# nadeemlab/DeepLIIF

Hardware: AMD Instinct MI355X
Metric: 512x512 tiles/s train-step (5G+5D) (higher is better)
Workload: dtype bf16; 1 GPU; DeepLIIF train step, 5x Resnet-9block G + 5x NLayerD(n=4), GAN+SmoothL1+Adam (BASELINE configs[2] per GPU); tile=512x512x3, batch_per_gpu=8, global_batch=8, norm=instance, precision_policy=bf16, parallelism=dp1, rccl_ranks=1, backend=nccl, streams=3

## Files before the change

deepliif_amd/_lib.py:

```python
import ctypes as C
import os

_HERE = os.path.dirname(os.path.abspath(__file__))
LIB_PATH = os.environ.get('DEEPLIIF_AMD_LIB') or os.path.join(_HERE, 'libdeepliif_hip.so')
LIB_PATH_F16 = os.environ.get('DEEPLIIF_AMD_LIB_F16') or os.path.join(_HERE, 'libdeepliif_hip_f16.so')
HALF_BF16, HALF_FP16 = 0, 1

DL_F32, DL_BF16 = 0, 1
PREC_BF16, PREC_BF16X3 = 1, 3
ACT_NONE, ACT_RELU, ACT_LRELU, ACT_TANH, ACT_SIGMOID = 0, 1, 2, 3, 4
PAD_ZERO, PAD_REFLECT, PAD_REPLICATE = 0, 1, 2
FOLD_SRC_F32 = 0x100
NORM_INSTANCE, NORM_BATCH = 0, 1
LOSS_BCE_LOGITS, LOSS_MSE, LOSS_SMOOTH_L1, LOSS_L1, LOSS_LINEAR = 0, 1, 2, 3, 4
MAX_TAPS, MAX_PHASES = 64, 4
WGRAD_MULTI_MAX = 24
DL_VERSION = 118

i32 = C.c_int32


class ConvDesc(C.Structure):
    _fields_ = [('N', i32), ('Hi', i32), ('Wi', i32), ('Ci', i32), ('in_pstride', i32),
                ('Ho', i32), ('Wo', i32), ('Co', i32), ('out_pstride', i32),
# ... 2 lines not shown
                ('phase_tap_begin', i32 * (MAX_PHASES + 1)), ('phase_kbase', i32 * MAX_PHASES),
                ('tap_dh', C.c_int8 * MAX_TAPS), ('tap_dw', C.c_int8 * MAX_TAPS),
                ('pad_mode', i32), ('w_kstride', i32), ('w_rows', i32), ('act', i32),
                ('in_dtype', i32), ('out_dtype', i32), ('prec', i32), ('splitk', i32), ('in_act', i32), ('bias_n', i32), ('raw_out', i32), ('ci_real', i32), ('in_split', i32)]



class ConvBnStats(C.Structure):
    _fields_ = [('y', C.c_void_p), ('y_pstride', C.c_int32), ('act', C.c_int32),
                ('mean', C.c_void_p), ('rstd', C.c_void_p), ('scale', C.c_void_p), ('shift', C.c_void_p)]

class WgradDesc(C.Structure):
    _fields_ = [('N', i32), ('Hp', i32), ('Wp', i32), ('CAp', i32), ('p_pstride', i32),
                ('Hq', i32), ('Wq', i32), ('CBp', i32), ('q_pstride', i32),
                ('KH', i32), ('KW', i32), ('step', i32), ('pad', i32), ('pad_mode', i32),
                ('CA', i32), ('CB', i32), ('dtype', i32), ('prec', i32), ('splitk', i32), ('accumulate', i32),
                ('q_act', i32), ('p_act', i32), ('pad_w', i32), ('stack_kw', i32), ('p_split', i32), ('q_split', i32)]


class WgradReduceEntry(C.Structure):
    _fields_ = [('slab', C.c_void_p), ('grad', C.c_void_p),
                ('splitk', i32), ('CAp', i32), ('CBp', i32), ('J', i32), ('CA', i32), ('CB', i32), ('KK', i32), ('accumulate', i32), ('stack_kw', i32),
                ('block0', i32), ('nblocks', i32), ('kstride', i32)]


class PackDesc(C.Structure):
    _fields_ = [('A', i32), ('B', i32), ('KH', i32), ('KW', i32), ('row_is_a', i32),
                ('rows_real', i32), ('rows_pad', i32), ('Cc', i32), ('Cc_pad', i32), ('n_phase', i32),
                ('phase_tap_begin', i32 * (MAX_PHASES + 1)), ('phase_kbase', i32 * MAX_PHASES),
                ('tap_kh', C.c_int8 * MAX_TAPS), ('tap_kw', C.c_int8 * MAX_TAPS), ('kstride', i32), ('stack_kw', i32)]


class NormDesc(C.Structure):
    _fields_ = [('N', i32), ('H', i32), ('W', i32), ('Cp', i32), ('C', i32),
                ('y_pstride', i32), ('z_pstride', i32), ('r_pstride', i32),
                ('dtype', i32), ('scope', i32), ('act', i32), ('eps', C.c_float), ('momentum', C.c_float), ('ext_nchunks', i32)]


class RenderThresh(C.Structure):
    _fields_ = [('size_lower', C.c_int64), ('size_upper', C.c_int64), ('marker', C.c_int64), ('od_lower', C.c_int64), ('od_upper', C.c_int64),
                ('has_size_upper', i32), ('has_marker', i32), ('has_od_lower', i32), ('has_od_upper', i32)]


class DropoutDesc(C.Structure):
    _fields_ = [('p', C.c_float), ('seed', C.c_uint64), ('seed_dev', C.c_void_p), ('call_index', C.c_uint32)]

# ... 30 lines not shown
    'dl_conv_wgrad_deferrable': (_i, [C.POINTER(WgradDesc)]),
    'dl_wgrad_slab_floats': (C.c_size_t, [C.POINTER(WgradDesc)]),
    'dl_conv_wgrad_slabs': (_i, [C.POINTER(WgradDesc), _vp, _vp, _vp, _vp, C.POINTER(WgradReduceEntry), _vp]),
    'dl_wgrad_reduce_batch': (_i, [_vp, _i, _i, _vp]),
    'dl_wgrad_plan': (_i, [C.POINTER(WgradDesc), C.POINTER(i32), C.POINTER(i32), C.POINTER(C.c_char_p)]),
    'dl_conv_wgrad_multi': (_i, [C.POINTER(WgradDesc), _i, _vp, _vp, _vp, _vp, C.POINTER(WgradReduceEntry), _vp]),
    'dl_pack_weights': (_i, [C.POINTER(PackDesc), _vp, _vp, _vp, _vp]),
    'dl_pack_job_bytes': (C.c_size_t, []),
    'dl_pack_job_fill': (_i, [C.POINTER(PackDesc), _vp, _vp, _vp, _vp]),
    'dl_pack_batch_blocks': (_i, [_vp, _i, _vp]),
    'dl_pack_weights_batch': (_i, [_vp, _vp, _i, _vp]),
    'dl_spectral_job_bytes': (C.c_size_t, []),
    'dl_spectral_scratch_floats': (C.c_size_t, [_i, _i]),
    'dl_spectral_job_fill': (_i, [_vp, _i, _i, _i, _i, _vp, _vp, _vp, _vp, _vp, _vp, _vp, _vp, _i64, _vp]),
    'dl_spectral_blocks': (_i, [_vp, _i, _i, _vp]),
    'dl_spectral_forward': (_i, [_vp, _i, _vp, _i, _vp, _i, _vp, _i, _vp, _i, _vp]),
    'dl_spectral_backward': (_i, [_vp, _i, _vp, _i, _vp, _i, _vp]),
    'dl_norm_ws_floats': (C.c_size_t, [C.POINTER(NormDesc)]),
    'dl_norm_forward': (_i, [C.POINTER(NormDesc), _vp, _vp, _vp, _vp, _vp, _vp, _vp, _vp, _vp, _vp, _vp, _vp, _vp, _vp]),
    'dl_norm_backward': (_i, [C.POINTER(NormDesc), _vp, _vp, _vp, _vp, _vp, _vp, _vp, _vp, _vp, _vp, _i, _vp, _vp, _vp, _vp]),
    'dl_norm_forward_dropout': (_i, [C.POINTER(NormDesc), _vp, _vp, _vp, _vp, _vp, _vp, _vp, _vp, _vp, _vp, _vp, _vp, _vp, _vp, C.POINTER(DropoutDesc)]),
    'dl_norm_backward_dropout': (_i, [C.POINTER(NormDesc), _vp, _vp, _vp, _vp, _vp, _vp, _vp, _vp, _vp, _vp, _i, _vp, _vp, _vp, _vp,
                                      C.POINTER(DropoutDesc)]),
    'dl_act_forward': (_i, [_i, _i, _vp, _i, _vp, _i, _i64, _i, _vp]),
    'dl_act_backward': (_i, [_i, _i, _vp, _i, _vp, _i, _vp, _i, _i64, _i, _vp]),
    'dl_dropout': (_i, [_i, _vp, _i, _vp, _i, _i64, _i, _f, C.c_uint64, _vp]),
    'dl_dropout_dev': (_i, [_i, _vp, _i, _vp, _i, _i64, _i, C.POINTER(DropoutDesc), _vp]),
    'dl_axpby': (_i, [_i, _f, _vp, _i, _f, _vp, _i, _vp, _i, _i64, _i, _vp]),
    'dl_gate_forward': (_i, [_i, _vp, _i, _vp, _i, _vp, _i, _i64, _i, _vp]),
    'dl_gate_backward': (_i, [_i, _vp, _i, _vp, _i, _vp, _i, _vp, _i, _vp, _i, _i64, _i, _vp]),
    'dl_copy_channels': (_i, [_i, _vp, _i, _i, _vp, _i, _i, _i64, _i, _i, _vp]),
    'dl_channel_sum': (_i, [_i, _vp, _i, _i64, _i, _i, _vp, _i, _vp, _vp]),
    'dl_nchw_to_nhwc': (_i, [_vp, _i, _i, _i, _i, _i, _vp, _i, _i, _i, _vp]),
    'dl_nhwc_to_nchw': (_i, [_i, _vp, _i, _i, _vp, _i, _i, _i, _i, _vp]),
    'dl_conv_narrow_supported': (_i, [_i, _i, _i, _i, _i, _i, _i, _i]),
    'dl_conv_narrow_forward': (_i, [_vp, _i, _i, _i, _i, _i, _vp, _i, _i, _i, _i, _i, _vp, _i, _vp, _i, _i, _vp]),
    'dl_conv_narrow_forward_x3': (_i, [_vp, _i, _i, _i, _i, _i, _vp, _vp, _i, _i, _i, _i, _i, _vp, _i, _vp, _i, _i, _vp]),
    'dl_shift_sum': (_i, [_vp, _i, _i, _i, _i, _i, _i, _i, _i, _vp, _i, _i, _vp, _i, _i, _vp]),
    'dl_shift_stack': (_i, [_i, _vp, _i, _i, _i, _i, _i, _i, _i, _i, _vp, _i, _vp]),
    'dl_reflect_fold': (_i, [_i, _vp, _i, _vp, _i, _i, _i, _i, _i, _i, _vp]),
    'dl_replicate_fold': (_i, [_i, _vp, _i, _vp, _i, _i, _i, _i, _i, _i, _vp]),
    'dl_loss_ws_floats': (C.c_size_t, []),
    'dl_loss': (_i, [_i, _i, _vp, _i, _vp, _i, _f, _i64, _i, _i, _vp, _vp, _i, _f, _vp, _vp]),
    'dl_loss_acc': (_i, [_i, _i, _vp, _i, _vp, _i, _f, _i64, _i, _i, _vp, _f, _i, _vp, _i, _f, _vp, _vp]),
    'dl_upsample2_nearest': (_i, [_i, _i, _vp, _i, _vp, _i, _i, _i, _i, _i, _vp]),
    'dl_kldiv_ws_floats': (C.c_size_t, []),
# ... 60 lines not shown
```

deepliif_amd/csrc/elementwise.hip:

```cpp
#include "common.h"

#define EW_BLOCKS(total) ((int)min((size_t)8192, ((size_t)(total) + 255) / 256))

template <typename T>
__global__ void __launch_bounds__(256) act_fwd_kernel(int act, const T *x, int x_ps, T *y, int y_ps, size_t npix, int Cp) {
    const int cvec = Cp / 8;
    const size_t total = npix * cvec;
    for (size_t i = blockIdx.x * (size_t)blockDim.x + threadIdx.x; i < total; i += (size_t)gridDim.x * blockDim.x) {
        const size_t p = i / cvec;
        const int c0 = (int)(i % cvec) * 8;
        float v[8];
        Vec8<T>::load(x + p * x_ps + c0, v);
#pragma unroll
        for (int k = 0; k < 8; ++k) v[k] = apply_act(act, v[k]);
        Vec8<T>::store(y + p * y_ps + c0, v);
    }
}
template <typename T>
__global__ void __launch_bounds__(256) act_bwd_kernel(int act, const T *dy, int dy_ps, const T *y, int y_ps, T *dx, int dx_ps, size_t npix,
                                                      int Cp) {
    const int cvec = Cp / 8;
    const size_t total = npix * cvec;
    for (size_t i = blockIdx.x * (size_t)blockDim.x + threadIdx.x; i < total; i += (size_t)gridDim.x * blockDim.x) {
        const size_t p = i / cvec;
// ... 210 lines not shown
                Vec8<T>::load(x + p * ps + (cbase + col) * 8, v);
#pragma unroll
                for (int k = 0; k < 8; ++k) s[k] += v[k];
            }
        }
#pragma unroll
        for (int k = 0; k < 8; ++k) red[tid * 9 + k] = s[k];
        __syncthreads();
        if (tid < tpp) {
            float a[8];
#pragma unroll
            for (int k = 0; k < 8; ++k) a[k] = 0.f;
            for (int r = 0; r < rows; ++r)
#pragma unroll
                for (int k = 0; k < 8; ++k) a[k] += red[(r * tpp + tid) * 9 + k];
#pragma unroll
            for (int k = 0; k < 8; ++k) part[(size_t)blockIdx.x * Cp + (cbase + tid) * 8 + k] = a[k];
        }
        __syncthreads();
    }
}
__global__ void __launch_bounds__(256) channel_sum_final_kernel(const float *part, int nblocks, int Cp, int C, float *out, int accumulate) {
    __shared__ float red[8][33];
    const int cl = threadIdx.x & 31, kl = threadIdx.x >> 5;
    const int c = blockIdx.x * 32 + cl;
    float s = 0.f;
    if (c < C)
        for (int b = kl; b < nblocks; b += 8) s += part[(size_t)b * Cp + c];
    red[kl][cl] = s;
    __syncthreads();
    if (kl == 0 && c < C) {
        double a = 0.0;
#pragma unroll
        for (int r = 0; r < 8; ++r) a += (double)red[r][cl];
        out[c] = (accumulate ? out[c] : 0.f) + (float)a;
    }
}
extern "C" int dl_channel_sum(int dtype, const void *x, int ps, int64_t npix, int Cp, int C, float *out, int accumulate, float *ws,
                              void *stream_) {
    hipStream_t stream = (hipStream_t)stream_;
    if (!x || !out || !ws || Cp % 8 || ps % 8) DL_FAIL("dl_channel_sum: bad argument (ws needs %d*Cp floats)", CS_BLOCKS);
    if (dtype == DL_F32) hipLaunchKernelGGL(channel_sum_partial_kernel<float>, dim3(CS_BLOCKS), dim3(256), 0, stream, (const float *)x, ps, (size_t)npix, Cp, ws);
    else hipLaunchKernelGGL(channel_sum_partial_kernel<bf16_t>, dim3(CS_BLOCKS), dim3(256), 0, stream, (const bf16_t *)x, ps, (size_t)npix, Cp, ws);
    DL_CHECK_LAUNCH("dl_channel_sum(partial)");
    hipLaunchKernelGGL(channel_sum_final_kernel, dim3((C + 31) / 32), dim3(256), 0, stream, ws, CS_BLOCKS, Cp, C, out, accumulate);
    DL_CHECK_LAUNCH("dl_channel_sum(final)");
    return 0;
}

#define LOSS_BLOCKS 512
extern "C" size_t dl_loss_ws_floats(void) { return LOSS_BLOCKS; }

template <typename T>
__global__ void __launch_bounds__(256) loss_kernel(int kind, const T *x, int x_ps, const T *target, int t_ps, float tconst, size_t npix, int C,
                                                   float inv_count, T *grad, int g_ps, float gscale, int Cp, float *part) {
    __shared__ float red[4];
    const size_t total = npix * C;
    float acc = 0.f;
    for (size_t i = blockIdx.x * (size_t)blockDim.x + threadIdx.x; i < total; i += (size_t)gridDim.x * blockDim.x) {
        const size_t p = i / C;
        const int c = (int)(i % C);
        const float v = load1<T>(x + p * x_ps + c);
        const float t = target ? load1<T>(target + p * t_ps + c) : tconst;
        float l, g;
        if (kind == DL_LOSS_BCE_LOGITS) {
            const float e = expf(-fabsf(v));
            l = fmaxf(v, 0.f) - v * t + log1pf(e);
            const float sig = v >= 0.f ? 1.f / (1.f + e) : e / (1.f + e);
            g = sig - t;
// ... 554 lines not shown
```

deepliif_amd/csrc/norm.hip:

```cpp
#include "common.h"

struct NormGeom {
    int N, HW, Cp, C;
    int nchunks, ppc;
};

static NormGeom make_geom(const dl_norm_desc *d) {
    NormGeom g;
    g.N = d->N; g.HW = d->H * d->W; g.Cp = d->Cp; g.C = d->C;
    int want = (1024 + d->N - 1) / d->N;
    int maxc = (g.HW + 63) / 64;
    g.nchunks = want < maxc ? want : maxc;
    if (g.nchunks < 1) g.nchunks = 1;
    g.ppc = (g.HW + g.nchunks - 1) / g.nchunks;
    g.nchunks = (g.HW + g.ppc - 1) / g.ppc;
    return g;
}

static NormGeom make_geom_fwd(const dl_norm_desc *d) {
    NormGeom g = make_geom(d);
    if (d->ext_nchunks > 0) { g.nchunks = d->ext_nchunks; g.ppc = 0; }
    return g;
}

// ... 343 lines not shown
        }
        if (bpart) {
#pragma unroll
            for (int k = 0; k < 8; ++k) bred[threadIdx.x * 9 + k] = bs[k];
            __syncthreads();
            if (threadIdx.x < tpp) {
                float a[8];
#pragma unroll
                for (int k = 0; k < 8; ++k) a[k] = 0.f;
                for (int r = 0; r < rows; ++r)
#pragma unroll
                    for (int k = 0; k < 8; ++k) a[k] += bred[(r * tpp + threadIdx.x) * 9 + k];
                float *o = bpart + ((size_t)(n * gridDim.x + blockIdx.x)) * g.Cp + (cbase + threadIdx.x) * 8;
#pragma unroll
                for (int k = 0; k < 8; ++k) o[k] = a[k];
            }
            __syncthreads();
        }
    }
}

__global__ void __launch_bounds__(1024) norm_bias_final_kernel(const float *part, int nparts, int Cp, int C, float *out) {
    __shared__ float red[32][33];
    const int cl = threadIdx.x & 31, kl = threadIdx.x >> 5;
    const int c = blockIdx.x * 32 + cl;
    float s = 0.f;
    if (c < C) {
        float acc[8] = {0.f, 0.f, 0.f, 0.f, 0.f, 0.f, 0.f, 0.f};
        int b = kl;
        for (; b + 7 * 32 < nparts; b += 8 * 32) {
#pragma unroll
            for (int u = 0; u < 8; ++u) acc[u] += part[(size_t)(b + u * 32) * Cp + c];
        }
        for (int u = 0; b < nparts; b += 32, ++u) acc[u & 7] += part[(size_t)b * Cp + c];
        s = ((acc[0] + acc[1]) + (acc[2] + acc[3])) + ((acc[4] + acc[5]) + (acc[6] + acc[7]));
    }
    red[kl][cl] = s;
    __syncthreads();
    if (kl == 0 && c < C) {
        double a = 0.0;
#pragma unroll
        for (int r = 0; r < 32; ++r) a += (double)red[r][cl];
        out[c] += (float)a;
    }
}

static dim3 apply_grid(const NormGeom &g) {
    const int cvec = g.Cp / 8;
    const int rows = 256 / (cvec < 256 ? cvec : 256);
    int bx = (g.HW + rows * 16 - 1) / (rows * 16);
    static const float mul = [] { const char *e = DL_DEV_ENV("DL_NORM_GRID_MUL"); const float v = e ? (float)atof(e) : 1.f; return v > 0.f ? v : 1.f; }();
    const int cap = kBiasPartRows / g.N > 1 ? kBiasPartRows / g.N : 1;
    int want = (int)(cap * mul);
    if (want > cap) want = cap;
    if (bx > want) bx = want;
    if (bx < 1) bx = 1;
    return dim3(bx, g.N);
}

#define DL_NORM_ACT_SWITCH(act_, LAUNCH)                  \
    switch (act_) {                                       \
        case DL_ACT_RELU: LAUNCH(DL_ACT_RELU); break;     \
        case DL_ACT_LRELU: LAUNCH(DL_ACT_LRELU); break;   \
        case DL_ACT_TANH: LAUNCH(DL_ACT_TANH); break;     \
        default: LAUNCH(DL_ACT_NONE); break;              \
    }

// ... 59 lines not shown
    }
    else if (d->dtype == DL_F32) { DL_NORM_ACT_SWITCH(d->act, DL_LAUNCH_APPLY_F32) }
    else { DL_NORM_ACT_SWITCH(d->act, DL_LAUNCH_APPLY_BF16) }
    DL_CHECK_LAUNCH("dl_norm_forward(apply)");
    return 0;
}

extern "C" int dl_norm_forward(const dl_norm_desc *d, const void *y, const float *gamma, const float *beta,
                               float *running_mean, float *running_var, float *mean, float *rstd, float *scale, float *shift,
                               const void *residual, void *z, float *ws, void *z_split, void *stream_) {
    return norm_forward_impl(d, y, gamma, beta, running_mean, running_var, mean, rstd, scale, shift, residual, z, ws, z_split, stream_, nullptr);
}

extern "C" int dl_norm_forward_dropout(const dl_norm_desc *d, const void *y, const float *gamma, const float *beta,
                                       float *running_mean, float *running_var, float *mean, float *rstd, float *scale, float *shift,
                                       const void *residual, void *z, float *ws, void *z_split, void *stream_, const dl_dropout_desc *drop) {
    if (check_drop(drop, "dl_norm_forward_dropout")) return -1;
    return norm_forward_impl(d, y, gamma, beta, running_mean, running_var, mean, rstd, scale, shift, residual, z, ws, z_split, stream_, drop);
}

static int norm_backward_impl(const dl_norm_desc *d, const void *dz, const void *y, const float *gamma,
                              const float *mean, const float *rstd, const float *scale, const float *shift,
                              void *dy, float *dgamma, float *dbeta, int accumulate_affine, float *dy_chansum, float *ws, void *dy_split,
                              void *stream_, const dl_dropout_desc *drop) {
    hipStream_t stream = (hipStream_t)stream_;
    if (check_desc(d, "dl_norm_backward")) return -1;
    if (drop && d->ext_nchunks > 0)
        DL_FAIL("dl_norm_backward_dropout: ext_nchunks = %d together with dropout is not supported (partials produced by a convolution were computed "
                "from the unmasked gradient)", d->ext_nchunks);
    if (dy_split && d->dtype != DL_F32) DL_FAIL("dl_norm_backward: the split copy belongs to the fp32 (strict) policy");
    if (!dz || !y || !mean || !rstd || !scale || !shift || !ws) DL_FAIL("dl_norm_backward: null argument");
    if (!dy && !dy_split) DL_FAIL("dl_norm_backward: dy may only be NULL when dy_split receives the result");
    const bool ext = d->ext_nchunks > 0;
    const NormGeom g = make_geom_fwd(d);
    float *part = ws;
    float *sums = ws + (size_t)g.N * g.nchunks * 2 * g.Cp;
    float *c1 = sums + (size_t)2 * g.N * g.Cp;
    float *c2 = c1 + (size_t)g.N * g.Cp;
    const int pblocks = g.N * g.nchunks;
    const int dz_ps = d->z_pstride, dy_ps = d->r_pstride;
#define DL_LAUNCH_BRED_F32(A) hipLaunchKernelGGL((norm_partial_kernel<float, 1, A>), dim3(pblocks), dim3(256), 0, stream, (const float *)y, \
                                                 d->y_pstride, (const float *)dz, dz_ps, g, mean, rstd, scale, shift, part)
#define DL_LAUNCH_BRED_BF16(A) hipLaunchKernelGGL((norm_partial_kernel<bf16_t, 1, A>), dim3(pblocks), dim3(256), 0, stream, (const bf16_t *)y, \
                                                  d->y_pstride, (const bf16_t *)dz, dz_ps, g, mean, rstd, scale, shift, part)
#define DL_LAUNCH_BRED_DROP_F32(A) hipLaunchKernelGGL((norm_partial_kernel<float, 1, A>), dim3(pblocks), dim3(256), 0, stream, (const float *)y, \
                                                      d->y_pstride, (const float *)dz, dz_ps, g, mean, rstd, scale, shift, part, da)
#define DL_LAUNCH_BRED_DROP_BF16(A) hipLaunchKernelGGL((norm_partial_kernel<bf16_t, 1, A>), dim3(pblocks), dim3(256), 0, stream, (const bf16_t *)y, \
                                                       d->y_pstride, (const bf16_t *)dz, dz_ps, g, mean, rstd, scale, shift, part, da)
    DropArgs da = {};
    if (drop) da = dl_drop_args(drop);
    if (drop) {
        if (d->dtype == DL_F32) { DL_NORM_ACT_SWITCH(d->act, DL_LAUNCH_BRED_DROP_F32) }
        else { DL_NORM_ACT_SWITCH(d->act, DL_LAUNCH_BRED_DROP_BF16) }
    }
    else if (ext) {  }
    else if (d->dtype == DL_F32) { DL_NORM_ACT_SWITCH(d->act, DL_LAUNCH_BRED_F32) }
    else { DL_NORM_ACT_SWITCH(d->act, DL_LAUNCH_BRED_BF16) }
    DL_CHECK_LAUNCH("dl_norm_backward(reduce)");
    if (d->scope == DL_NORM_INSTANCE && !dgamma) {
        hipLaunchKernelGGL(norm_chunk_sum_kernel<2>, dim3((g.Cp + 31) / 32, g.N), dim3(1024), 0, stream, part, g, sums, d->eps, c1, c2, nullptr, nullptr, nullptr, nullptr);
        DL_CHECK_LAUNCH("dl_norm_backward(chunk sums + finalize)");
    } else {
        hipLaunchKernelGGL(norm_chunk_sum_kernel<0>, dim3((g.Cp + 31) / 32, g.N), dim3(1024), 0, stream, part, g, sums, d->eps, nullptr, nullptr, nullptr, nullptr, nullptr, nullptr);
        DL_CHECK_LAUNCH("dl_norm_backward(chunk sums)");
        hipLaunchKernelGGL(norm_bwd_finalize_kernel, dim3((g.Cp + 255) / 256), dim3(256), 0, stream, sums, g, d->scope, c1, c2, dgamma, dbeta,
                           accumulate_affine);
        DL_CHECK_LAUNCH("dl_norm_backward(finalize)");
    }
    float *bpart = dy_chansum ? c2 + (size_t)g.N * g.Cp : nullptr;
    const dim3 blocks = apply_grid(g);
#define DL_LAUNCH_BAPPLY_F32(A) hipLaunchKernelGGL((norm_bwd_apply_kernel<float, A>), blocks, dim3(256), 0, stream, (const float *)dz, dz_ps, \
                                                   (const float *)y, d->y_pstride, gamma, mean, rstd, scale, shift, c1, c2, (float *)dy, dy_ps, g, bpart, \
                                                   (float *)dy_split, d->Cp)
#define DL_LAUNCH_BAPPLY_BF16(A) hipLaunchKernelGGL((norm_bwd_apply_kernel<bf16_t, A>), blocks, dim3(256), 0, stream, (const bf16_t *)dz, dz_ps, \
                                                    (const bf16_t *)y, d->y_pstride, gamma, mean, rstd, scale, shift, c1, c2, (bf16_t *)dy, dy_ps, g, bpart, \
                                                    (float *)nullptr, 0)
#define DL_LAUNCH_BAPPLY_DROP_F32(A) hipLaunchKernelGGL((norm_bwd_apply_kernel<float, A>), blocks, dim3(256), 0, stream, (const float *)dz, dz_ps, \
                                                        (const float *)y, d->y_pstride, gamma, mean, rstd, scale, shift, c1, c2, (float *)dy, dy_ps, g, bpart, \
                                                        (float *)dy_split, d->Cp, da)
#define DL_LAUNCH_BAPPLY_DROP_BF16(A) hipLaunchKernelGGL((norm_bwd_apply_kernel<bf16_t, A>), blocks, dim3(256), 0, stream, (const bf16_t *)dz, dz_ps, \
                                                         (const bf16_t *)y, d->y_pstride, gamma, mean, rstd, scale, shift, c1, c2, (bf16_t *)dy, dy_ps, g, bpart, \
                                                         (float *)nullptr, 0, da)
    if (drop) {
        if (d->dtype == DL_F32) { DL_NORM_ACT_SWITCH(d->act, DL_LAUNCH_BAPPLY_DROP_F32) }
        else { DL_NORM_ACT_SWITCH(d->act, DL_LAUNCH_BAPPLY_DROP_BF16) }
    }
    else if (d->dtype == DL_F32) { DL_NORM_ACT_SWITCH(d->act, DL_LAUNCH_BAPPLY_F32) }
    else { DL_NORM_ACT_SWITCH(d->act, DL_LAUNCH_BAPPLY_BF16) }
    DL_CHECK_LAUNCH("dl_norm_backward(apply)");
    if (dy_chansum) {
        hipLaunchKernelGGL(norm_bias_final_kernel, dim3((g.C + 31) / 32), dim3(1024), 0, stream, bpart, (int)(blocks.x * blocks.y), g.Cp, g.C, dy_chansum);
        DL_CHECK_LAUNCH("dl_norm_backward(bias sum)");
    }
    return 0;
}

extern "C" int dl_norm_backward(const dl_norm_desc *d, const void *dz, const void *y, const float *gamma,
                                const float *mean, const float *rstd, const float *scale, const float *shift,
                                void *dy, float *dgamma, float *dbeta, int accumulate_affine, float *dy_chansum, float *ws, void *dy_split,
                                void *stream_) {
    return norm_backward_impl(d, dz, y, gamma, mean, rstd, scale, shift, dy, dgamma, dbeta, accumulate_affine, dy_chansum, ws, dy_split, stream_, nullptr);
}

extern "C" int dl_norm_backward_dropout(const dl_norm_desc *d, const void *dz, const void *y, const float *gamma,
                                        const float *mean, const float *rstd, const float *scale, const float *shift,
                                        void *dy, float *dgamma, float *dbeta, int accumulate_affine, float *dy_chansum, float *ws, void *dy_split,
                                        void *stream_, const dl_dropout_desc *drop) {
    if (check_drop(drop, "dl_norm_backward_dropout")) return -1;
    return norm_backward_impl(d, dz, y, gamma, mean, rstd, scale, shift, dy, dgamma, dbeta, accumulate_affine, dy_chansum, ws, dy_split, stream_, drop);
}
```

deepliif_amd/ops.py:

```python
from __future__ import annotations

import ctypes as C
import os
import contextlib
import threading
from typing import Optional

import torch

from . import _lib as L
from .geometry import (GatherPlan, NUM_CUS, WGRAD_C4_PARTS, choose_splitk, choose_wgrad_batch_splitk, choose_wgrad_splitk, fill_conv_desc, fill_pack_desc,
                       wgrad_batch_shape, wgrad_c4_ok, wgrad_fast_path)


def dl_dtype(t: torch.Tensor) -> int:
    if t.dtype == torch.float32:
        return L.DL_F32
    if t.dtype == torch.bfloat16 or t.dtype == torch.float16:
        return L.DL_BF16
    raise TypeError(f'engine tensors are fp32 or bf16 / fp16, got {t.dtype}')


def pstride(t: torch.Tensor) -> int:
    assert t.dim() == 4 and t.stride(3) == 1, 'NHWC view with unit channel stride expected'
    ps = t.stride(2)
    assert t.stride(1) == t.shape[2] * ps and t.stride(0) == t.shape[1] * t.shape[2] * ps, 'pixels must be densely strided'
    return ps


_SHARED_SCRATCH = os.environ.get('DL_SHARED_SCRATCH', '0') == '1'
_BNSTATS = os.environ.get('DL_BNSTATS', '0') == '1'
_CONV_ADD = os.environ.get('DL_CONV_ADD', '1') != '0'
_NO_WGRAD_C4 = os.environ.get('DL_NO_WGRAD_C4', '0') == '1'
_NO_X3_GLDS = os.environ.get('DL_NO_X3_GLDS') is not None
_X3_ACTS = (L.ACT_NONE, L.ACT_RELU, L.ACT_LRELU)
_SPLIT_ONLY_GRAD = os.environ.get('DL_NO_SPLIT_ONLY_GRAD', '0') != '1'
_NO_C4_X3 = 'DL_NO_C4_X3' in os.environ
_WGRAD_DEFER = os.environ.get('DL_WGRAD_DEFER', '1') != '0'
_WGRAD_ARENA_MB = int(os.environ.get('DL_WGRAD_ARENA_MB', '256'))
_WGRAD_BATCH = os.environ.get('DL_WGRAD_BATCH', '1') != '0'
_NO_NARROW_ROLL = os.environ.get('DL_NO_NARROW_ROLL', '0') == '1'
_SHARED_STATE: dict = {}


_FAST_STREAM = hasattr(torch._C, '_cuda_getCurrentRawStream') and hasattr(torch._C, '_cuda_getDevice')


def _current_stream_handle(dev_index=None) -> int:
    if _FAST_STREAM and torch.cuda.is_initialized():
        return torch._C._cuda_getCurrentRawStream(torch._C._cuda_getDevice() if dev_index is None else dev_index)
    return torch.cuda.current_stream(dev_index).cuda_stream if dev_index is not None else torch.cuda.current_stream().cuda_stream


class Workspace:

    def __init__(self):
        self._tls = threading.local()
        self._branch_ids = set()
        self._branch_lock = threading.Lock()

    def _thread_state(self):
# ... 355 lines not shown
        nslab = int(self.lib.dl_wgrad_slab_floats(C.byref(d)))
        if deferring and self.lib.dl_conv_wgrad_deferrable(C.byref(d)):
            self._wgrad_deferred(WS._state(), d, P, Q, grad, nslab)
            return
        slab = WS.get('wgrad_slab', nslab, P.device)
        self.check(self.lib.dl_conv_wgrad(C.byref(d), _ptr(P), _ptr(Q), _ptr(grad), _ptr(slab), _stream()), 'dl_conv_wgrad')

    def wgrad_defer_begin(self):
        st = WS._thread_state()
        st['defer_depth'] = st.get('defer_depth', 0) + 1

    def wgrad_defer_end(self):
        st = WS._thread_state()
        try:
            if st.get('defer_depth', 0) == 1:
                self.wgrad_flush_all()
        finally:
            st['defer_depth'] = max(0, st.get('defer_depth', 0) - 1)

    def wgrad_abandon(self):
        st = WS._thread_state()
        for sub in [st] + WS.stream_states():
            sub['defer_pending'], sub['defer_queue'], sub['defer_blocks'], sub['defer_off'] = [], [], 0, 0
            sub['defer_grads'] = set()
        st['defer_depth'] = 0

    def wgrad_flush_all(self):
        self.wgrad_flush()
        for sub in WS.stream_states():
            if sub.get('defer_pending') or sub.get('defer_queue'):
                with torch.cuda.stream(sub['stream_obj']):
                    self.wgrad_flush()

    def _arena_region(self, st, need: int, device):
        arena = st.get('defer_arena')
        if arena is not None and st.get('defer_off', 0) + need > arena.numel():
            self._reduce_pending(st)
        if arena is None or arena.numel() < need or arena.device != device:
            self._reduce_pending(st)
            if arena is not None:
                Workspace.realloc_generation += 1
            arena = torch.empty(max(need, _WGRAD_ARENA_MB * (1 << 18)), dtype=torch.float32, device=device)
            st['defer_arena'], st['defer_off'] = arena, 0
        off = st.get('defer_off', 0)
        st['defer_off'] = off + need
        return arena[off:off + need]

    def _wgrad_queued(self, st, d, P, Q, grad, tiles, ksteps):
        gp = grad.data_ptr()
        if gp in st.setdefault('defer_grads', set()):
            self.wgrad_flush()
        st['defer_grads'].add(gp)
        d.splitk = choose_wgrad_batch_splitk(tiles, ksteps)
# ... 28 lines not shown
                    e.block0 = st.get('defer_blocks', 0)
                    st['defer_blocks'] = e.block0 + e.nblocks
                    pend.append(e)

    def _wgrad_deferred(self, st, d, P, Q, grad, nslab):
        gp = grad.data_ptr()
        need = (nslab + 63) // 64 * 64
        if gp in st.setdefault('defer_grads', set()):
            self.wgrad_flush()
        slab = self._arena_region(st, need, P.device)
        e = L.WgradReduceEntry()
        self.check(self.lib.dl_conv_wgrad_slabs(C.byref(d), _ptr(P), _ptr(Q), _ptr(grad), _ptr(slab), C.byref(e), _stream()), 'dl_conv_wgrad_slabs')
        e.block0 = st.get('defer_blocks', 0)
        st['defer_blocks'] = e.block0 + e.nblocks
        st['defer_grads'].add(gp)
        st.setdefault('defer_pending', []).append(e)

    def wgrad_flush(self):
        st = WS._state()
        self._launch_queued(st)
        self._reduce_pending(st)
        st['defer_grads'] = set()

    def _reduce_pending(self, st):
        pend = st.get('defer_pending')
        if not pend:
            st['defer_off'] = 0
            return
        arena = st['defer_arena']
        tab = (L.WgradReduceEntry * len(pend))(*pend)
        key = bytes(tab)
        cache = st.setdefault('defer_tables', {})
        dev_tab = cache.get(key)
        if dev_tab is None:
            if len(cache) >= 512:
                cache.clear()
            dev_tab = torch.frombuffer(bytearray(key), dtype=torch.uint8).to(arena.device)
            cache[key] = dev_tab
        total = st['defer_blocks']
        st['defer_pending'], st['defer_blocks'], st['defer_off'] = [], 0, 0
        _LAUNCH.dev = arena.device
        self.check(self.lib.dl_wgrad_reduce_batch(_ptr(dev_tab), len(pend), total, _stream()), 'dl_wgrad_reduce_batch')

    supports_split = os.environ.get('DL_NO_SPLIT_COPY') is None

    def conv_takes_split(self, x, prec, in_act, pad_mode) -> bool:
        return (self.supports_split and not _NO_X3_GLDS and x.dtype == torch.float32 and prec == L.PREC_BF16X3 and in_act == L.ACT_NONE)
# ... 39 lines not shown
        d.ext_nchunks = ext_nchunks
        if not ext_nchunks:
            WS.bump_norm_token()
        stats = torch.empty(4, y.shape[0], y.shape[3], dtype=torch.float32, device=y.device)
        ws = WS.get('norm_ws', self.lib.dl_norm_ws_floats(C.byref(d)), y.device)
        args = (C.byref(d), _ptr(y), _ptr(gamma), _ptr(beta), _ptr(running_mean), _ptr(running_var),
                _ptr(stats[0]), _ptr(stats[1]), _ptr(stats[2]), _ptr(stats[3]), _ptr(residual), _ptr(z) if store_z else None,
                _ptr(ws), _ptr(z_split), _stream())
        if dropout is None:
            self.check(self.lib.dl_norm_forward(*args), 'dl_norm_forward')
        else:
            self.check(self.lib.dl_norm_forward_dropout(*args, C.byref(self._dropout_desc(dropout))), 'dl_norm_forward_dropout')
        return stats

    def norm_backward(self, dz, y, dy, stats, C_real, scope, act, gamma, dgamma, dbeta, dy_chansum=None, ext_nchunks=0, dy_split=None, store_dy=True,
                      dropout=None):
        _need_cuda(dz, y, dy, dy_chansum, dy_split)
        assert store_dy or dy_split is not None
        assert dy_split is None or (dy_split.is_contiguous() and dy_split.dtype == torch.float32 and dy_split.shape == dy.shape)
        d = self._norm_desc(y, C_real, scope, act, -1.0, pstride(dz), pstride(dy))
        d.ext_nchunks = ext_nchunks
        WS.bump_norm_token()
        ws = WS.get('norm_ws', self.lib.dl_norm_ws_floats(C.byref(d)), y.device)
        args = (C.byref(d), _ptr(dz), _ptr(y), _ptr(gamma), _ptr(stats[0]), _ptr(stats[1]), _ptr(stats[2]),
                _ptr(stats[3]), _ptr(dy) if store_dy else None, _ptr(dgamma), _ptr(dbeta), 1, _ptr(dy_chansum), _ptr(ws), _ptr(dy_split), _stream())
        if dropout is None:
            self.check(self.lib.dl_norm_backward(*args), 'dl_norm_backward')
        else:
            self.check(self.lib.dl_norm_backward_dropout(*args, C.byref(self._dropout_desc(dropout))), 'dl_norm_backward_dropout')

    def act_forward(self, act, x, y):
        _need_cuda(x, y)
        npix = x.shape[0] * x.shape[1] * x.shape[2]
        self.check(self.lib.dl_act_forward(act, dl_dtype(x), _ptr(x), pstride(x), _ptr(y), pstride(y), npix, x.shape[3], _stream()), 'dl_act_forward')

    def act_backward(self, act, dy, y, dx):
        _need_cuda(dy, y, dx)
        npix = y.shape[0] * y.shape[1] * y.shape[2]
        self.check(self.lib.dl_act_backward(act, dl_dtype(y), _ptr(dy), pstride(dy), _ptr(y), pstride(y), _ptr(dx), pstride(dx), npix,
                                         y.shape[3], _stream()), 'dl_act_backward')

    def dropout(self, x, y, p, seed):
        _need_cuda(x, y)
        npix = x.shape[0] * x.shape[1] * x.shape[2]
        self.check(self.lib.dl_dropout(dl_dtype(x), _ptr(x), pstride(x), _ptr(y), pstride(y), npix, x.shape[3], float(p), int(seed) & (2 ** 64 - 1),
                                    _stream()), 'dl_dropout')
# ... 11 lines not shown
                                  _ptr(out), pstride(out), npix, a.shape[3], _stream()), 'dl_axpby')

    def gate_forward(self, x, psi, out):
        _need_cuda(x, psi, out)
        npix = x.shape[0] * x.shape[1] * x.shape[2]
        self.check(self.lib.dl_gate_forward(dl_dtype(x), _ptr(x), pstride(x), _ptr(psi), pstride(psi), _ptr(out), pstride(out), npix, x.shape[3], _stream()),
                'dl_gate_forward')

    def gate_backward(self, g, x, psi, dx, dpsi):
        _need_cuda(g, x, psi, dx, dpsi)
        npix = x.shape[0] * x.shape[1] * x.shape[2]
        self.check(self.lib.dl_gate_backward(dl_dtype(x), _ptr(g), pstride(g), _ptr(x), pstride(x), _ptr(psi), pstride(psi), _ptr(dx),
                                          pstride(dx) if dx is not None else 8, _ptr(dpsi), pstride(dpsi), npix, x.shape[3], _stream()), 'dl_gate_backward')

    def copy_channels(self, src, s_c0, dst, d_c0, nch, accumulate=False):
        _need_cuda(src, dst)
        npix = src.shape[0] * src.shape[1] * src.shape[2]
        self.check(self.lib.dl_copy_channels(dl_dtype(src), _ptr(src), pstride(src), s_c0, _ptr(dst), pstride(dst), d_c0, npix, nch,
                                          1 if accumulate else 0, _stream()), 'dl_copy_channels')

    def channel_sum(self, x, C_real, out, accumulate):
        _need_cuda(x, out)
        npix = x.shape[0] * x.shape[1] * x.shape[2]
        ws = WS.get('csum_ws', 256 * x.shape[3], x.device)
        self.check(self.lib.dl_channel_sum(dl_dtype(x), _ptr(x), pstride(x), npix, x.shape[3], C_real, _ptr(out), 1 if accumulate else 0,
                                        _ptr(ws), _stream()), 'dl_channel_sum')

    def nchw_to_nhwc(self, src, dst, c0, zero_pad_to):
        _need_cuda(src, dst)
        assert src.dtype == torch.float32 and src.is_contiguous()
        n, c, h, w = src.shape
        self.check(self.lib.dl_nchw_to_nhwc(_ptr(src), n, c, h, w, dl_dtype(dst), _ptr(dst), pstride(dst), c0, zero_pad_to, _stream()),
                'dl_nchw_to_nhwc')

    def nhwc_to_nchw(self, src, c0, dst):
        _need_cuda(src, dst)
        assert dst.dtype == torch.float32 and dst.is_contiguous()
        n, c, h, w = dst.shape
        self.check(self.lib.dl_nhwc_to_nchw(dl_dtype(src), _ptr(src), pstride(src), c0, _ptr(dst), n, c, h, w, _stream()), 'dl_nhwc_to_nchw')

    def conv_narrow_supported(self, x, cin_p, cout, k, pad, pad_mode, act=L.ACT_NONE) -> bool:
        return act in (L.ACT_NONE, L.ACT_TANH) and bool(self.lib.dl_conv_narrow_supported(dl_dtype(x), cin_p, pstride(x), cout, k, k, pad, pad_mode)) and not _NO_NARROW_ROLL

    def conv_narrow_forward(self, packed, x, out, cout, k, pad, bias, act):
        _need_cuda(x, out, bias, packed.hi)
        n, h, w, cp = x.shape
# ... 196 lines not shown
```

include/deepliif_hip.h:

```cpp
#ifndef DEEPLIIF_HIP_H
#define DEEPLIIF_HIP_H

#include <stddef.h>
#include <stdint.h>

#ifdef __cplusplus
extern "C" {
#endif

#define DL_VERSION 118

enum { DL_F32 = 0, DL_BF16 = 1 };
enum { DL_HALF_BF16 = 0, DL_HALF_FP16 = 1 };
enum { DL_PREC_BF16 = 1, DL_PREC_BF16X3 = 3 };
enum { DL_ACT_NONE = 0, DL_ACT_RELU = 1, DL_ACT_LRELU = 2, DL_ACT_TANH = 3,
       DL_ACT_SIGMOID = 4 };
enum { DL_PAD_ZERO = 0, DL_PAD_REFLECT = 1,
       DL_PAD_REPLICATE = 2 };
enum { DL_NORM_INSTANCE = 0, DL_NORM_BATCH = 1 };
enum { DL_LOSS_BCE_LOGITS = 0, DL_LOSS_MSE = 1, DL_LOSS_SMOOTH_L1 = 2, DL_LOSS_L1 = 3,
       DL_LOSS_LINEAR = 4 };

#define DL_MAX_TAPS 64
#define DL_MAX_PHASES 4
// ... 148 lines not shown
                    float *running_mean, float *running_var,
                    float *mean, float *rstd, float *scale, float *shift,
                    const void *residual, void *z, float *ws, void *z_split, void *stream);

int dl_norm_backward(const dl_norm_desc *d, const void *dz, const void *y, const float *gamma,
                     const float *mean, const float *rstd, const float *scale, const float *shift,
                     void *dy, float *dgamma, float *dbeta, int accumulate_affine, float *dy_chansum, float *ws, void *dy_split, void *stream);

typedef struct dl_dropout_desc {
    float p;
    uint64_t seed;
    const uint64_t *seed_dev;
    uint32_t call_index;
} dl_dropout_desc;
int dl_norm_forward_dropout(const dl_norm_desc *d, const void *y, const float *gamma, const float *beta,
                            float *running_mean, float *running_var,
                            float *mean, float *rstd, float *scale, float *shift,
                            const void *residual, void *z, float *ws, void *z_split, void *stream, const dl_dropout_desc *drop);
int dl_norm_backward_dropout(const dl_norm_desc *d, const void *dz, const void *y, const float *gamma,
                             const float *mean, const float *rstd, const float *scale, const float *shift,
                             void *dy, float *dgamma, float *dbeta, int accumulate_affine, float *dy_chansum, float *ws, void *dy_split, void *stream,
                             const dl_dropout_desc *drop);

int dl_act_forward(int act, int dtype, const void *x, int x_pstride, void *y, int y_pstride, int64_t npix, int Cp, void *stream);
int dl_act_backward(int act, int dtype, const void *dy, int dy_pstride, const void *y, int y_pstride,
                    void *dx, int dx_pstride, int64_t npix, int Cp, void *stream);
int dl_gate_forward(int dtype, const void *x, int x_pstride, const void *psi, int psi_pstride, void *out, int out_pstride, int64_t npix, int Cp,
                    void *stream);
int dl_gate_backward(int dtype, const void *g, int g_pstride, const void *x, int x_pstride, const void *psi, int psi_pstride, void *dx,
                     int dx_pstride, void *dpsi, int dpsi_pstride, int64_t npix, int Cp, void *stream);
int dl_dropout(int dtype, const void *x, int x_pstride, void *y, int y_pstride, int64_t npix, int Cp, float p, uint64_t seed, void *stream);
int dl_dropout_dev(int dtype, const void *x, int x_pstride, void *y, int y_pstride, int64_t npix, int Cp, const dl_dropout_desc *drop, void *stream);
int dl_axpby(int dtype, float alpha, const void *a, int a_pstride, float beta, const void *b, int b_pstride,
             void *out, int out_pstride, int64_t npix, int Cp, void *stream);
int dl_copy_channels(int dtype, const void *src, int src_pstride, int src_c0, void *dst, int dst_pstride, int dst_c0,
                     int64_t npix, int C, int accumulate, void *stream);
int dl_channel_sum(int dtype, const void *x, int pstride, int64_t npix, int Cp, int C, float *out, int accumulate,
                   float *ws, void *stream);
int dl_nchw_to_nhwc(const float *src, int N, int C, int H, int W, int dtype, void *dst, int dst_pstride, int dst_c0,
                    int zero_pad_to, void *stream);
int dl_nhwc_to_nchw(int dtype, const void *src, int src_pstride, int src_c0, float *dst, int N, int C, int H, int W,
                    void *stream);

size_t dl_loss_ws_floats(void);
int dl_loss(int kind, int dtype, const void *x, int x_pstride, const void *target, int t_pstride, float target_const,
            int64_t npix, int C, int Cp, float *loss_out, void *grad, int g_pstride, float grad_scale,
// ... 86 lines not shown
```

Baseline: 119.0 tiles/s.

## Defer bias-gradient row reductions into one batched reduce kernel per flush

When wgrad deferral is active, the norm backward and channel_sum calls now write per-block partial rows into the deferral arena and queue a table entry. They no longer launch a separate final reduction kernel for each bias. A single batched kernel looks up each block's entry by binary search and reduces all queued bias gradients at wgrad flush time. This is meant to cut many small kernel launches, at the cost of arena space, host-side table building and caching, and extra flush bookkeeping for gradient aliasing.

```diff
diff --git a/deepliif_amd/_lib.py b/deepliif_amd/_lib.py
--- a/deepliif_amd/_lib.py
+++ b/deepliif_amd/_lib.py
@@ -48,6 +48,14 @@
     _fields_ = [('slab', C.c_void_p), ('grad', C.c_void_p),
                 ('splitk', i32), ('CAp', i32), ('CBp', i32), ('J', i32), ('CA', i32), ('CB', i32), ('KK', i32), ('accumulate', i32), ('stack_kw', i32),
                 ('block0', i32), ('nblocks', i32), ('kstride', i32)]
+
+
+class BiasReduceEntry(C.Structure):
+    _fields_ = [('rows', C.c_void_p), ('out', C.c_void_p), ('nrows', i32), ('Cp', i32), ('C', i32), ('kind', i32), ('accumulate', i32), ('block0', i32)]
+
+
+BIAS_ROWS_NORM, BIAS_ROWS_CHANNEL_SUM = 0, 1
+CHANNEL_SUM_ROWS = 256
 
 
 class PackDesc(C.Structure):
@@ -124,6 +132,11 @@
     'dl_norm_forward_dropout': (_i, [C.POINTER(NormDesc), _vp, _vp, _vp, _vp, _vp, _vp, _vp, _vp, _vp, _vp, _vp, _vp, _vp, _vp, C.POINTER(DropoutDesc)]),
     'dl_norm_backward_dropout': (_i, [C.POINTER(NormDesc), _vp, _vp, _vp, _vp, _vp, _vp, _vp, _vp, _vp, _vp, _i, _vp, _vp, _vp, _vp,
                                       C.POINTER(DropoutDesc)]),
+    'dl_norm_bias_rows': (_i, [C.POINTER(NormDesc)]),
+    'dl_norm_backward_rows': (_i, [C.POINTER(NormDesc), _vp, _vp, _vp, _vp, _vp, _vp, _vp, _vp, _vp, _vp, _i, _vp, _vp, _vp, _vp,
+                                   C.POINTER(DropoutDesc)]),
+    'dl_channel_sum_rows': (_i, [_i, _vp, _i, _i64, _i, _vp, _vp]),
+    'dl_bias_reduce_batch': (_i, [_vp, _i, _i, _vp]),
     'dl_act_forward': (_i, [_i, _i, _vp, _i, _vp, _i, _i64, _i, _vp]),
     'dl_act_backward': (_i, [_i, _i, _vp, _i, _vp, _i, _vp, _i, _i64, _i, _vp]),
     'dl_dropout': (_i, [_i, _vp, _i, _vp, _i, _i64, _i, _f, C.c_uint64, _vp]),
diff --git a/deepliif_amd/csrc/bias_rows.h b/deepliif_amd/csrc/bias_rows.h
--- /dev/null
+++ b/deepliif_amd/csrc/bias_rows.h
@@ -0,0 +1,43 @@
+#pragma once
+
+__device__ __forceinline__ void bias_rows_sum32(const float *part, int nparts, int Cp, int C, float *out, int cblock, float (*red)[33]) {
+    const int cl = threadIdx.x & 31, kl = threadIdx.x >> 5;
+    const int c = cblock * 32 + cl;
+    float s = 0.f;
+    if (c < C) {
+        float acc[8] = {0.f, 0.f, 0.f, 0.f, 0.f, 0.f, 0.f, 0.f};
+        int b = kl;
+        for (; b + 7 * 32 < nparts; b += 8 * 32) {
+#pragma unroll
+            for (int u = 0; u < 8; ++u) acc[u] += part[(size_t)(b + u * 32) * Cp + c];
+        }
+        for (int u = 0; b < nparts; b += 32, ++u) acc[u & 7] += part[(size_t)b * Cp + c];
+        s = ((acc[0] + acc[1]) + (acc[2] + acc[3])) + ((acc[4] + acc[5]) + (acc[6] + acc[7]));
+    }
+    red[kl][cl] = s;
+    __syncthreads();
+    if (kl == 0 && c < C) {
+        double a = 0.0;
+#pragma unroll
+        for (int r = 0; r < 32; ++r) a += (double)red[r][cl];
+        out[c] += (float)a;
+    }
+}
+
+__device__ __forceinline__ void bias_rows_sum8(const float *part, int nblocks, int Cp, int C, float *out, int accumulate, int cblock, float (*red)[33]) {
+    const int cl = threadIdx.x & 31, kl = threadIdx.x >> 5;
+    const int c = cblock * 32 + cl;
+    if (kl < 8) {
+        float s = 0.f;
+        if (c < C)
+            for (int b = kl; b < nblocks; b += 8) s += part[(size_t)b * Cp + c];
+        red[kl][cl] = s;
+    }
+    __syncthreads();
+    if (kl == 0 && c < C) {
+        double a = 0.0;
+#pragma unroll
+        for (int r = 0; r < 8; ++r) a += (double)red[r][cl];
+        out[c] = (accumulate ? out[c] : 0.f) + (float)a;
+    }
+}
diff --git a/deepliif_amd/csrc/elementwise.hip b/deepliif_amd/csrc/elementwise.hip
--- a/deepliif_amd/csrc/elementwise.hip
+++ b/deepliif_amd/csrc/elementwise.hip
@@ -1,4 +1,5 @@
 #include "common.h"
+#include "bias_rows.h"
 
 #define EW_BLOCKS(total) ((int)min((size_t)8192, ((size_t)(total) + 255) / 256))
 
@@ -256,19 +257,7 @@
 }
 __global__ void __launch_bounds__(256) channel_sum_final_kernel(const float *part, int nblocks, int Cp, int C, float *out, int accumulate) {
     __shared__ float red[8][33];
-    const int cl = threadIdx.x & 31, kl = threadIdx.x >> 5;
-    const int c = blockIdx.x * 32 + cl;
-    float s = 0.f;
-    if (c < C)
-        for (int b = kl; b < nblocks; b += 8) s += part[(size_t)b * Cp + c];
-    red[kl][cl] = s;
-    __syncthreads();
-    if (kl == 0 && c < C) {
-        double a = 0.0;
-#pragma unroll
-        for (int r = 0; r < 8; ++r) a += (double)red[r][cl];
-        out[c] = (accumulate ? out[c] : 0.f) + (float)a;
-    }
+    bias_rows_sum8(part, nblocks, Cp, C, out, accumulate, blockIdx.x, red);
 }
 extern "C" int dl_channel_sum(int dtype, const void *x, int ps, int64_t npix, int Cp, int C, float *out, int accumulate, float *ws,
                               void *stream_) {
@@ -279,6 +268,15 @@
     DL_CHECK_LAUNCH("dl_channel_sum(partial)");
     hipLaunchKernelGGL(channel_sum_final_kernel, dim3((C + 31) / 32), dim3(256), 0, stream, ws, CS_BLOCKS, Cp, C, out, accumulate);
     DL_CHECK_LAUNCH("dl_channel_sum(final)");
+    return 0;
+}
+extern "C" int dl_channel_sum_rows(int dtype, const void *x, int ps, int64_t npix, int Cp, float *rows, void *stream_) {
+    hipStream_t stream = (hipStream_t)stream_;
+    static_assert(CS_BLOCKS == DL_CHANNEL_SUM_ROWS, "include/deepliif_hip.h promises this many rows");
+    if (!x || !rows || Cp % 8 || ps % 8) DL_FAIL("dl_channel_sum_rows: bad argument (rows needs %d*Cp floats)", CS_BLOCKS);
+    if (dtype == DL_F32) hipLaunchKernelGGL(channel_sum_partial_kernel<float>, dim3(CS_BLOCKS), dim3(256), 0, stream, (const float *)x, ps, (size_t)npix, Cp, rows);
+    else hipLaunchKernelGGL(channel_sum_partial_kernel<bf16_t>, dim3(CS_BLOCKS), dim3(256), 0, stream, (const bf16_t *)x, ps, (size_t)npix, Cp, rows);
+    DL_CHECK_LAUNCH("dl_channel_sum_rows");
     return 0;
 }
 
diff --git a/deepliif_amd/csrc/norm.hip b/deepliif_amd/csrc/norm.hip
--- a/deepliif_amd/csrc/norm.hip
+++ b/deepliif_amd/csrc/norm.hip
@@ -1,4 +1,5 @@
 #include "common.h"
+#include "bias_rows.h"
 
 struct NormGeom {
     int N, HW, Cp, C;
@@ -389,27 +390,28 @@
 
 __global__ void __launch_bounds__(1024) norm_bias_final_kernel(const float *part, int nparts, int Cp, int C, float *out) {
     __shared__ float red[32][33];
-    const int cl = threadIdx.x & 31, kl = threadIdx.x >> 5;
-    const int c = blockIdx.x * 32 + cl;
-    float s = 0.f;
-    if (c < C) {
-        float acc[8] = {0.f, 0.f, 0.f, 0.f, 0.f, 0.f, 0.f, 0.f};
-        int b = kl;
-        for (; b + 7 * 32 < nparts; b += 8 * 32) {
-#pragma unroll
-            for (int u = 0; u < 8; ++u) acc[u] += part[(size_t)(b + u * 32) * Cp + c];
-        }
-        for (int u = 0; b < nparts; b += 32, ++u) acc[u & 7] += part[(size_t)b * Cp + c];
-        s = ((acc[0] + acc[1]) + (acc[2] + acc[3])) + ((acc[4] + acc[5]) + (acc[6] + acc[7]));
-    }
-    red[kl][cl] = s;
-    __syncthreads();
-    if (kl == 0 && c < C) {
-        double a = 0.0;
-#pragma unroll
-        for (int r = 0; r < 32; ++r) a += (double)red[r][cl];
-        out[c] += (float)a;
-    }
+    bias_rows_sum32(part, nparts, Cp, C, out, blockIdx.x, red);
+}
+
+__global__ void __launch_bounds__(1024) bias_reduce_batch_kernel(const dl_bias_reduce_entry *tab, int n) {
+    __shared__ float red[32][33];
+    int lo = 0, hi = n - 1;
+    const int b = blockIdx.x;
+    while (lo < hi) {
+        const int mid = (lo + hi + 1) >> 1;
+        if (tab[mid].block0 <= b) lo = mid; else hi = mid - 1;
+    }
+    const dl_bias_reduce_entry e = tab[lo];
+    if (e.kind == DL_BIAS_ROWS_NORM) bias_rows_sum32(e.rows, e.nrows, e.Cp, e.C, e.out, b - e.block0, red);
+    else bias_rows_sum8(e.rows, e.nrows, e.Cp, e.C, e.out, e.accumulate, b - e.block0, red);
+}
+
+extern "C" int dl_bias_reduce_batch(const dl_bias_reduce_entry *table_dev, int count, int total_blocks, void *stream_) {
+    hipStream_t stream = (hipStream_t)stream_;
+    if (!table_dev || count <= 0 || total_blocks <= 0) DL_FAIL("dl_bias_reduce_batch: empty table");
+    hipLaunchKernelGGL(bias_reduce_batch_kernel, dim3(total_blocks), dim3(1024), 0, stream, table_dev, count);
+    DL_CHECK_LAUNCH("dl_bias_reduce_batch");
+    return 0;
 }
 
 static dim3 apply_grid(const NormGeom &g) {
@@ -515,9 +517,10 @@
 static int norm_backward_impl(const dl_norm_desc *d, const void *dz, const void *y, const float *gamma,
                               const float *mean, const float *rstd, const float *scale, const float *shift,
                               void *dy, float *dgamma, float *dbeta, int accumulate_affine, float *dy_chansum, float *ws, void *dy_split,
-                              void *stream_, const dl_dropout_desc *drop) {
+                              void *stream_, const dl_dropout_desc *drop, float *bias_rows = nullptr) {
     hipStream_t stream = (hipStream_t)stream_;
     if (check_desc(d, "dl_norm_backward")) return -1;
+    if (bias_rows && dy_chansum) DL_FAIL("dl_norm_backward_rows: the channel sums of dy are either summed now (dy_chansum) or left as rows (bias_rows), not both");
     if (drop && d->ext_nchunks > 0)
         DL_FAIL("dl_norm_backward_dropout: ext_nchunks = %d together with dropout is not supported (partials produced by a convolution were computed "
                 "from the unmasked gradient)", d->ext_nchunks);
@@ -560,7 +563,7 @@
                            accumulate_affine);
         DL_CHECK_LAUNCH("dl_norm_backward(finalize)");
     }
-    float *bpart = dy_chansum ? c2 + (size_t)g.N * g.Cp : nullptr;
+    float *bpart = bias_rows ? bias_rows : dy_chansum ? c2 + (size_t)g.N * g.Cp : nullptr;
     const dim3 blocks = apply_grid(g);
 #define DL_LAUNCH_BAPPLY_F32(A) hipLaunchKernelGGL((norm_bwd_apply_kernel<float, A>), blocks, dim3(256), 0, stream, (const float *)dz, dz_ps, \
                                                    (const float *)y, d->y_pstride, gamma, mean, rstd, scale, shift, c1, c2, (float *)dy, dy_ps, g, bpart, \
@@ -602,3 +605,18 @@
     if (check_drop(drop, "dl_norm_backward_dropout")) return -1;
     return norm_backward_impl(d, dz, y, gamma, mean, rstd, scale, shift, dy, dgamma, dbeta, accumulate_affine, dy_chansum, ws, dy_split, stream_, drop);
 }
+
+extern "C" int dl_norm_bias_rows(const dl_norm_desc *d) {
+    if (check_desc(d, "dl_norm_bias_rows")) return -1;
+    const dim3 blocks = apply_grid(make_geom_fwd(d));
+    return (int)(blocks.x * blocks.y);
+}
+
+extern "C" int dl_norm_backward_rows(const dl_norm_desc *d, const void *dz, const void *y, const float *gamma,
+                                     const float *mean, const float *rstd, const float *scale, const float *shift,
+                                     void *dy, float *dgamma, float *dbeta, int accumulate_affine, float *bias_rows, float *ws, void *dy_split,
+                                     void *stream_, const dl_dropout_desc *drop) {
+    if (!bias_rows) DL_FAIL("dl_norm_backward_rows: null bias_rows");
+    if (drop && check_drop(drop, "dl_norm_backward_rows")) return -1;
+    return norm_backward_impl(d, dz, y, gamma, mean, rstd, scale, shift, dy, dgamma, dbeta, accumulate_affine, nullptr, ws, dy_split, stream_, drop, bias_rows);
+}
diff --git a/deepliif_amd/ops.py b/deepliif_amd/ops.py
--- a/deepliif_amd/ops.py
+++ b/deepliif_amd/ops.py
@@ -37,6 +37,7 @@
 _SPLIT_ONLY_GRAD = os.environ.get('DL_NO_SPLIT_ONLY_GRAD', '0') != '1'
 _NO_C4_X3 = 'DL_NO_C4_X3' in os.environ
 _WGRAD_DEFER = os.environ.get('DL_WGRAD_DEFER', '1') != '0'
+_BIAS_DEFER = os.environ.get('DL_BIAS_DEFER', '1') != '0'
 _WGRAD_ARENA_MB = int(os.environ.get('DL_WGRAD_ARENA_MB', '256'))
 _WGRAD_BATCH = os.environ.get('DL_WGRAD_BATCH', '1') != '0'
 _NO_NARROW_ROLL = os.environ.get('DL_NO_NARROW_ROLL', '0') == '1'
@@ -438,13 +439,14 @@
         st = WS._thread_state()
         for sub in [st] + WS.stream_states():
             sub['defer_pending'], sub['defer_queue'], sub['defer_blocks'], sub['defer_off'] = [], [], 0, 0
+            sub['bias_pending'], sub['bias_blocks'] = [], 0
             sub['defer_grads'] = set()
         st['defer_depth'] = 0
 
     def wgrad_flush_all(self):
         self.wgrad_flush()
         for sub in WS.stream_states():
-            if sub.get('defer_pending') or sub.get('defer_queue'):
+            if sub.get('defer_pending') or sub.get('defer_queue') or sub.get('bias_pending'):
                 with torch.cuda.stream(sub['stream_obj']):
                     self.wgrad_flush()
 
@@ -519,7 +521,50 @@
         self._reduce_pending(st)
         st['defer_grads'] = set()
 
+    def _bias_deferring(self, out) -> bool:
+        return _BIAS_DEFER and out is not None and WS._thread_state().get('defer_depth', 0) > 0
+
+    def _bias_region(self, st, out, nrows: int, cp: int):
+        gp = out.data_ptr()
+        if gp in st.setdefault('defer_grads', set()):
+            self.wgrad_flush()
+        rows = self._arena_region(st, (nrows * cp + 63) // 64 * 64, out.device)
+        st['defer_grads'].add(gp)
+        return rows
+
+    def _bias_pending(self, st, rows, out, nrows: int, cp: int, c_real: int, kind: int, accumulate: bool):
+        e = L.BiasReduceEntry()
+        e.rows, e.out, e.nrows, e.Cp, e.C, e.kind, e.accumulate = rows.data_ptr(), out.data_ptr(), nrows, cp, c_real, kind, 1 if accumulate else 0
+        e.block0 = st.get('bias_blocks', 0)
+        st['bias_blocks'] = e.block0 + (c_real + 31) // 32
+        st.setdefault('bias_pending', []).append(e)
+
+    def _flush_immediate_target(self, out):
+        if out is not None:
+            st = WS._state()
+            if out.data_ptr() in st.get('defer_grads', ()):
+                self.wgrad_flush()
+
+    def _reduce_bias_pending(self, st):
+        pend = st.get('bias_pending')
+        if not pend:
+            return
+        arena = st['defer_arena']
+        key = bytes((L.BiasReduceEntry * len(pend))(*pend))
+        cache = st.setdefault('bias_tables', {})
+        dev_tab = cache.get(key)
+        if dev_tab is None:
+            if len(cache) >= 512:
+                cache.clear()
+            dev_tab = torch.frombuffer(bytearray(key), dtype=torch.uint8).to(arena.device)
+            cache[key] = dev_tab
+        total = st['bias_blocks']
+        st['bias_pending'], st['bias_blocks'] = [], 0
+        _LAUNCH.dev = arena.device
+        self.check(self.lib.dl_bias_reduce_batch(_ptr(dev_tab), len(pend), total, _stream()), 'dl_bias_reduce_batch')
+
     def _reduce_pending(self, st):
+        self._reduce_bias_pending(st)
         pend = st.get('defer_pending')
         if not pend:
             st['defer_off'] = 0
@@ -605,6 +650,19 @@
         d.ext_nchunks = ext_nchunks
         WS.bump_norm_token()
         ws = WS.get('norm_ws', self.lib.dl_norm_ws_floats(C.byref(d)), y.device)
+        if self._bias_deferring(dy_chansum):
+            st = WS._state()
+            nrows = int(self.lib.dl_norm_bias_rows(C.byref(d)))
+            if nrows < 0:
+                self.check(nrows, 'dl_norm_bias_rows')
+            rows = self._bias_region(st, dy_chansum, nrows, d.Cp)
+            self.check(self.lib.dl_norm_backward_rows(
+                C.byref(d), _ptr(dz), _ptr(y), _ptr(gamma), _ptr(stats[0]), _ptr(stats[1]), _ptr(stats[2]), _ptr(stats[3]), _ptr(dy) if store_dy else None,
+                _ptr(dgamma), _ptr(dbeta), 1, _ptr(rows), _ptr(ws), _ptr(dy_split), _stream(),
+                C.byref(self._dropout_desc(dropout)) if dropout is not None else None), 'dl_norm_backward_rows')
+            self._bias_pending(st, rows, dy_chansum, nrows, d.Cp, C_real, L.BIAS_ROWS_NORM, True)
+            return
+        self._flush_immediate_target(dy_chansum)
         args = (C.byref(d), _ptr(dz), _ptr(y), _ptr(gamma), _ptr(stats[0]), _ptr(stats[1]), _ptr(stats[2]),
                 _ptr(stats[3]), _ptr(dy) if store_dy else None, _ptr(dgamma), _ptr(dbeta), 1, _ptr(dy_chansum), _ptr(ws), _ptr(dy_split), _stream())
         if dropout is None:
@@ -662,6 +720,13 @@
     def channel_sum(self, x, C_real, out, accumulate):
         _need_cuda(x, out)
         npix = x.shape[0] * x.shape[1] * x.shape[2]
+        if self._bias_deferring(out):
+            st = WS._state()
+            rows = self._bias_region(st, out, L.CHANNEL_SUM_ROWS, x.shape[3])
+            self.check(self.lib.dl_channel_sum_rows(dl_dtype(x), _ptr(x), pstride(x), npix, x.shape[3], _ptr(rows), _stream()), 'dl_channel_sum_rows')
+            self._bias_pending(st, rows, out, L.CHANNEL_SUM_ROWS, x.shape[3], C_real, L.BIAS_ROWS_CHANNEL_SUM, accumulate)
+            return
+        self._flush_immediate_target(out)
         ws = WS.get('csum_ws', 256 * x.shape[3], x.device)
         self.check(self.lib.dl_channel_sum(dl_dtype(x), _ptr(x), pstride(x), npix, x.shape[3], C_real, _ptr(out), 1 if accumulate else 0,
                                         _ptr(ws), _stream()), 'dl_channel_sum')
diff --git a/include/deepliif_hip.h b/include/deepliif_hip.h
--- a/include/deepliif_hip.h
+++ b/include/deepliif_hip.h
@@ -194,6 +194,22 @@
                              void *dy, float *dgamma, float *dbeta, int accumulate_affine, float *dy_chansum, float *ws, void *dy_split, void *stream,
                              const dl_dropout_desc *drop);
 
+enum { DL_BIAS_ROWS_NORM = 0,
+       DL_BIAS_ROWS_CHANNEL_SUM = 1 };
+#define DL_CHANNEL_SUM_ROWS 256
+typedef struct dl_bias_reduce_entry {
+    const float *rows;
+    float *out;
+    int32_t nrows, Cp, C, kind, accumulate, block0;
+} dl_bias_reduce_entry;
+int dl_norm_bias_rows(const dl_norm_desc *d);
+int dl_norm_backward_rows(const dl_norm_desc *d, const void *dz, const void *y, const float *gamma,
+                          const float *mean, const float *rstd, const float *scale, const float *shift,
+                          void *dy, float *dgamma, float *dbeta, int accumulate_affine, float *bias_rows, float *ws, void *dy_split, void *stream,
+                          const dl_dropout_desc *drop);
+int dl_channel_sum_rows(int dtype, const void *x, int pstride, int64_t npix, int Cp, float *rows, void *stream);
+int dl_bias_reduce_batch(const dl_bias_reduce_entry *table_dev, int count, int total_blocks, void *stream);
+
 int dl_act_forward(int act, int dtype, const void *x, int x_pstride, void *y, int y_pstride, int64_t npix, int Cp, void *stream);
 int dl_act_backward(int act, int dtype, const void *dy, int dy_pstride, const void *y, int y_pstride,
                     void *dx, int dx_pstride, int64_t npix, int Cp, void *stream);
```

Result: no change. 119.1 tiles/s, median of 6 (+0.2%).
